# AllanYangZhou/midGPT

Measured on AMD Instinct MI355X. Metric: tokens_per_sec, higher is better.
Workload: dtype bf16; 1 GPU; model=openwebtext_xl-gpt-1311M, global_batch=128, seq_len=1024, parallelism=dp1, g_accum_iters=2, remat=False

## Files before the change

midgpt_amd/models/gpt.py:

```python
from __future__ import annotations

import contextlib
import math
import os

import torch
import torch.nn as nn
import torch.nn.functional as F

from midgpt_amd import ops
from midgpt_amd.config import GPTConfig
from midgpt_amd.ops.reference import rope_tables


_SCOPES = os.environ.get("MIDGPT_SCOPES") == "1"


def _scope(name):
    return torch.profiler.record_function(name) if _SCOPES \
        else contextlib.nullcontext()


def _init_linear_(w: torch.Tensor, in_features: int, generator=None):
    nn.init.trunc_normal_(w, mean=0.0, std=1.0, a=-2.0, b=2.0, generator=generator)
    with torch.no_grad():
        w.mul_(1.0 / math.sqrt(in_features))


class Linear(nn.Module):

    def __init__(self, in_features: int, out_features: int, generator=None):
        super().__init__()
        self.weight = nn.Parameter(torch.empty(out_features, in_features))
        _init_linear_(self.weight, in_features, generator)

    def forward(self, x):
        return F.linear(x, self.weight.to(x.dtype))


class CausalSelfAttention(nn.Module):
    def __init__(self, config: GPTConfig, generator=None):
        super().__init__()
        D, H = config.n_embd, config.n_head
        assert D % H == 0
        self.n_head, self.n_embd = H, D
        self.head_dim = D // H
        self.c_attn = Linear(D, 3 * D, generator)
        self.c_proj = Linear(D, D, generator)
        self.q_ln_weight = nn.Parameter(torch.ones(self.head_dim))
        self.k_ln_weight = nn.Parameter(torch.ones(self.head_dim))
        self.dropout = config.dropout
        self.attn_dropout = nn.Dropout(config.dropout)
        self.resid_dropout = nn.Dropout(config.dropout)

    def forward(self, x, sin, cos):
        with _scope("causal_sa"):
            return self._forward(x, sin, cos)

    def _forward(self, x, sin, cos):
        B, T, D = x.shape
        qkv = self.c_attn(x).view(B, T, 3, self.n_head, self.head_dim)
        if (self.dropout > 0.0 and self.training
                and os.environ.get("MIDGPT_ATTN_DROPOUT_REF") == "1"):
            from midgpt_amd.ops import reference as refops
            q, k, v = ops.qkv_prep(qkv, self.q_ln_weight, self.k_ln_weight,
                                   sin[:T], cos[:T])
            o = refops.causal_attention(q, k, v, self.dropout, True)
            o = o.transpose(1, 2).reshape(B, T, D)
        else:
            o = ops.qkv_attention(qkv, self.q_ln_weight, self.k_ln_weight,
                                  sin[:T], cos[:T],
                                  self.dropout if self.training else 0.0)
        return self.resid_dropout(self.c_proj(o))


class MLP(nn.Module):
    def __init__(self, config: GPTConfig, generator=None):
        super().__init__()
        D = config.n_embd
        self.c_fc = Linear(D, 4 * D, generator)
        self.c_proj = Linear(4 * D, D, generator)
        self.dropout = nn.Dropout(config.dropout)

    def forward(self, x):
        with _scope("mlp"):
            if (x.is_cuda and x.dtype == torch.bfloat16 and ops.have_ext()
                    and os.environ.get("MIDGPT_FUSED_MLP") == "1"):
                return self.dropout(ops.fused_mlp(x, self.c_fc.weight,
                                                  self.c_proj.weight))
            if os.environ.get("MIDGPT_GELU_HIP") == "1":
                return self.dropout(self.c_proj(ops.gelu(self.c_fc(x))))
            return self.dropout(
                self.c_proj(F.gelu(self.c_fc(x), approximate="tanh")))


class Block(nn.Module):

    def __init__(self, config: GPTConfig, generator=None):
        super().__init__()
        self.attn = CausalSelfAttention(config, generator)
        self.mlp = MLP(config, generator)

    def forward(self, x, sin, cos):
        with _scope("block"):
            x = x + self.attn(ops.rmsnorm(x, None, 1e-6), sin, cos)
            x = x + self.mlp(ops.rmsnorm(x, None, 1e-6))
            return x

    def forward_pending(self, x, pending, sin, cos):
        with _scope("block"):
            if pending is None:
                h = ops.rmsnorm(x, None, 1e-6)
            else:
                x, h = ops.add_rmsnorm(x, pending, 1e-6)
            x, h = ops.add_rmsnorm(x, self.attn(h, sin, cos), 1e-6)
            return x, self.mlp(h)


class GPT(nn.Module):
# ... 56 lines not shown
```

midgpt_amd/ops/__init__.py:

```python
from __future__ import annotations

import math
import os

import torch

from midgpt_amd.ops import ref_backend

_C = None
_C_ERR: str | None = None

BACKEND_API = (
    "rmsnorm_fwd", "rmsnorm_bwd", "qkv_prep_fwd", "qkv_prep_bwd",
    "attn_fwd", "attn_bwd", "attn_fwd_dropout", "attn_bwd_dropout",
    "gelu_fwd", "gelu_bwd", "embedding_bwd", "ce_fwd", "ce_bwd",
    "adamw_step", "kv_append", "attn_decode",
)
RAGGED_API = ("kv_append_ragged", "attn_decode_ragged")
SAMPLING_API = ("sample_tokens",)
SLOT_API = ("kv_append_slots", "attn_decode_slots", "sample_tokens_rows")
PAGED_API = ("kv_append_paged", "attn_decode_paged", "kv_store_paged")


def _try_load_ext():
    global _C, _C_ERR
    if _C is not None:
        return _C
    try:
        import importlib
        _C = importlib.import_module("midgpt_amd.ops._C")
    except Exception as e:
        _C_ERR = repr(e)
        _C = None
    return _C


_try_load_ext()


def have_ext() -> bool:
    return _C is not None


def _use_hip(*tensors) -> bool:
    on_gpu = any(t.is_cuda for t in tensors if isinstance(t, torch.Tensor))
    if not on_gpu:
        return False
    if os.environ.get("MIDGPT_FORCE_REF") == "1":
        return False
    if _C is None:
        raise RuntimeError(
            "midgpt_amd HIP extension (midgpt_amd/ops/_C) is not built but a GPU "
            f"tensor reached a hot op. Build it with __graft_entry__.build(). "
            f"Import error: {_C_ERR}")
    return True


def _backend(*tensors):
    return _C if _use_hip(*tensors) else ref_backend


class _RMSNorm(torch.autograd.Function):
    @staticmethod
    def forward(ctx, x, weight, eps):
        shp = x.shape
        x2d = x.reshape(-1, shp[-1])
        y, invrms = _backend(x).rmsnorm_fwd(x2d.contiguous(), weight, eps)
        ctx.save_for_backward(x2d, invrms, *( [weight] if weight is not None else [] ))
        ctx.eps = eps
        ctx.has_w = weight is not None
        return y.reshape(shp)

    @staticmethod
    def backward(ctx, dy):
        saved = ctx.saved_tensors
        x2d, invrms = saved[0], saved[1]
        weight = saved[2] if ctx.has_w else None
        dy2d = dy.reshape(x2d.shape)
        dx, dw = _backend(x2d).rmsnorm_bwd(dy2d.contiguous(), x2d.contiguous(),
                                           weight, invrms, ctx.eps)
        return dx.reshape(dy.shape), dw, None


def rmsnorm(x, weight=None, eps: float = 1e-6):
    return _RMSNorm.apply(x, weight, eps)


def glue_unfused() -> bool:
    return os.environ.get("MIDGPT_GLUE_UNFUSED") == "1"


class _AddRMSNorm(torch.autograd.Function):
    @staticmethod
    def forward(ctx, x, r, eps):
        shp = x.shape
        D = shp[-1]
        s, y, invrms = _C.add_rmsnorm_fwd(x.reshape(-1, D).contiguous(),
                                          r.reshape(-1, D).contiguous(), eps)
        ctx.save_for_backward(s, invrms)
        ctx.set_materialize_grads(False)
        return s.view(shp), y.view(shp)

    @staticmethod
    def backward(ctx, ds, dy):
# ... 454 lines not shown
        if x.dtype != torch.bfloat16 or x.numel() % 8:
            impl = ref_backend
        return impl.gelu_fwd(x.contiguous())

    @staticmethod
    def backward(ctx, dy):
        (x,) = ctx.saved_tensors
        impl = _backend(x)
        if x.dtype != torch.bfloat16 or x.numel() % 8:
            impl = ref_backend
        return impl.gelu_bwd(dy.contiguous(), x.contiguous())


def gelu(x):
    return _Gelu.apply(x)


class _Embedding(torch.autograd.Function):
    @staticmethod
    def forward(ctx, idx, weight):
        ctx.save_for_backward(idx)
        ctx.V = weight.shape[0]
        return weight[idx]

    @staticmethod
    def backward(ctx, dy):
        (idx,) = ctx.saved_tensors
        dy2d = dy.reshape(-1, dy.shape[-1])
        impl = _backend(dy)
        if dy.dtype != torch.bfloat16:
            impl = ref_backend
        return None, impl.embedding_bwd(dy2d.contiguous(), idx.reshape(-1), ctx.V)


def embedding(idx, weight):
    return _Embedding.apply(idx, weight)


class _CrossEntropy(torch.autograd.Function):
    @staticmethod
    def forward(ctx, logits, targets):
        loss_sum, lse = _backend(logits).ce_fwd(logits, targets)
        ctx.save_for_backward(logits, targets, lse)
        return loss_sum / logits.shape[0]

    @staticmethod
    def backward(ctx, dloss):
        logits, targets, lse = ctx.saved_tensors
        dlogits = _backend(logits).ce_bwd(logits, targets, lse,
                                          dloss.float().reshape(1))
        return dlogits, None


def cross_entropy(logits, targets):
    return _CrossEntropy.apply(logits, targets)


class _FusedMLP(torch.autograd.Function):
    @staticmethod
    def forward(ctx, x2d, w1, w2):
        h = torch.mm(x2d, w1.t())
        g = torch.nn.functional.gelu(h, approximate="tanh")
        y = torch.mm(g, w2.t())
        ctx.save_for_backward(x2d, w1, w2, h, g)
        return y

    @staticmethod
    def backward(ctx, dy):
        x2d, w1, w2, h, g = ctx.saved_tensors
        dy = dy.contiguous()
        dh = _C.matmul_dgelu(dy, w2, h)
        dw2 = torch.mm(dy.t(), g)
        dx = torch.mm(dh, w1)
        dw1 = torch.mm(dh.t(), x2d)
        return dx, dw1, dw2


def fused_mlp(x, w1, w2):
    shp = x.shape
    y = _FusedMLP.apply(x.reshape(-1, shp[-1]).contiguous(), w1, w2)
    return y.reshape(*shp[:-1], w2.shape[0])


def adamw_step(master: torch.Tensor, grad: torch.Tensor, m: torch.Tensor,
               v: torch.Tensor, out_bf16: torch.Tensor | None,
               *, lr: float, beta1: float, beta2: float, eps: float,
               wd_over_peak_lr: float, grad_scale: float, clip_norm: float,
               sq_sum: torch.Tensor, step: int):
    _backend(master).adamw_step(master, grad, m, v,
                                out_bf16 if out_bf16 is not None
                                else master.new_empty(0, dtype=torch.bfloat16),
                                out_bf16 is not None, sq_sum,
                                lr, beta1, beta2, eps, wd_over_peak_lr,
                                grad_scale, clip_norm, step)
```

midgpt_amd/ops/csrc/bindings.cpp:

```cpp
#include <torch/extension.h>
#include <hip/hip_runtime.h>
#include <c10/hip/HIPGuard.h>
#include <c10/hip/HIPStream.h>

#include <algorithm>
#include <climits>
#include <type_traits>
#include <vector>

static hipStream_t cur_stream() { return c10::hip::getCurrentHIPStream().stream(); }

template <typename... P, typename... A>
static void launch(void (*kernel)(P...), dim3 grid, int block, size_t smem, A... args) {
  if (grid.x == 0 || grid.y == 0 || grid.z == 0) return;
  if (smem > 64 * 1024) {
    hipError_t e = hipFuncSetAttribute(reinterpret_cast<const void*>(kernel),
                                       hipFuncAttributeMaxDynamicSharedMemorySize, (int)smem);
    TORCH_CHECK(e == hipSuccess, "cannot raise dynamic LDS to ", smem, " bytes: ",
                hipGetErrorString(e));
  }
  hipLaunchKernelGGL(kernel, grid, dim3(block), smem, cur_stream(), static_cast<P>(args)...);
  hipError_t e = hipGetLastError();
  TORCH_CHECK(e == hipSuccess, "HIP launch failed: ", hipGetErrorString(e));
}
// ... 503 lines not shown

std::vector<torch::Tensor> attn_fwd_packed(torch::Tensor q, torch::Tensor k,
                                           torch::Tensor v, double p, int64_t seed) {
  Call c("attn_fwd_packed", q);
  const AttnQK a = attn_qk(c, q, k);
  AttnStrides sv;
  const u16* vp = packed_or_plain_v(c, a, v, &sv);
  auto o = torch::empty({a.B, a.T, a.H, a.C}, q.options());
  auto lse = torch::empty({a.B, a.H, a.T}, q.options().dtype(torch::kFloat));
  attn_fwd_launch(a, vp, sv, fresh<u16>(o), strides_bthc(a.H, a.T, a.C), fresh<float>(lse),
                  drop_if(p, seed));
  return {o, lse};
}

std::vector<torch::Tensor> attn_bwd_packed(torch::Tensor dO, torch::Tensor q,
                                           torch::Tensor k, torch::Tensor v,
                                           torch::Tensor o, torch::Tensor lse,
                                           torch::Tensor dqkv, double p, int64_t seed,
                                           bool stage_do) {
  Call c("attn_bwd_packed", dO);
  const AttnQK a = attn_qk(c, q, k);
  const int B = a.B, H = a.H, T = a.T, C = a.C;
  AttnStrides sv;
  const u16* vp = packed_or_plain_v(c, a, v, &sv);
  u16* dvp = c.bf16_out(dqkv, "dqkv", {B, T, 3, H, C}) + 2L * H * C;
  const u16 *dop = c.bf16(dO, "dO", {B, T, H, C}), *op = c.bf16(o, "o", {B, T, H, C});
  const float* lsep = c.f32(lse, "lse", flat(a.rows()));
  const AttnStrides sdv = strides_qkv_slot(H, T, C), so = strides_bthc(H, T, C);
  torch::Tensor do_copy;
  if (stage_do) do_copy = torch::empty_like(q);
  return attn_bwd_launch(a, dop, so, vp, sv, op, so, lsep, dvp, sdv, drop_if(p, seed),
                         stage_do ? fresh<u16>(do_copy) : nullptr);
}

torch::Tensor embedding_bwd(torch::Tensor dy, torch::Tensor idx, long V) {
  Call c("embedding_bwd", dy);
  const u16* dyp = c.bf16(dy, "dy", {ANY, ANY});
  long N = dy.size(0);
  int D = c.dim(dy, 1);
  const long* ip = c.i64(idx, "idx", {N});
  TORCH_CHECK(D % 8 == 0, "embedding_bwd: D % 8 == 0");
  if (D % 64 == 0) {
    auto sorted_perm = idx.sort();
    auto sorted = std::get<0>(sorted_perm).contiguous();
    auto perm = std::get<1>(sorted_perm).contiguous();
    auto dw = torch::zeros({V, (long)D}, dy.options());
    const int wpb = 4;
    long grid = (N + wpb - 1) / wpb;
    for (int d0 = 0; d0 < D; d0 += 2048)
      launch(embed_bwd_sorted_kernel, grid, wpb * 64, 0, dyp, fresh<long>(sorted),
             fresh<long>(perm), fresh<u16>(dw), N, D, d0);
    return dw;
  }
  auto dw32 = torch::zeros({V, (long)D}, dy.options().dtype(torch::kFloat));
  long grid = std::min(N, (long)4096);
  launch(embed_bwd_scatter_kernel, grid, 256, 0, dyp, ip, fresh<float>(dw32), N, D);
  auto dw = torch::empty({V, (long)D}, dy.options());
  long n = V * (long)D;
  long cgrid = std::min((n / 4 + 255) / 256 + 1, (long)4096);
  launch(f32_to_bf16_kernel, cgrid, 256, 0, fresh<float>(dw32), fresh<u16>(dw), n);
  return dw;
}

torch::Tensor gelu_fwd(torch::Tensor x) {
  Call c("gelu_fwd", x);
  long n = x.numel();
  const u16* xp = c.bf16(x, "x", flat(n));
  TORCH_CHECK(n % 8 == 0, "gelu_fwd: numel % 8 == 0 required");
  auto y = torch::empty_like(x);
  long grid = std::min((n / 8 + 255) / 256 + 1, (long)8192);
  launch(gelu_fwd_bf16, grid, 256, 0, xp, fresh<u16>(y), n);
  return y;
}

torch::Tensor gelu_bwd(torch::Tensor dy, torch::Tensor x) {
  Call c("gelu_bwd", dy);
  long n = x.numel();
  const u16 *xp = c.bf16(x, "x", flat(n)), *dyp = c.bf16(dy, "dy", flat(n));
  TORCH_CHECK(n % 8 == 0, "gelu_bwd: numel % 8 == 0 required");
  auto dx = torch::empty_like(x);
  long grid = std::min((n / 8 + 255) / 256 + 1, (long)8192);
  launch(gelu_bwd_bf16, grid, 256, 0, dyp, xp, fresh<u16>(dx), n);
  return dx;
}

static int64_t decode_caches(const Call& c, const torch::Tensor& k_cache,
                             const torch::Tensor& v_cache, int B, int H, int C, u16** kp,
                             u16** vp, int* pool = nullptr) {
  TORCH_CHECK(C == 64 || C == 128, c.who, ": head dim 64 or 128 (got ", C, ")");
  *kp = c.bf16_out(k_cache, "k_cache", {pool ? ANY : B, H, ANY, C});
  *vp = c.bf16_out(v_cache, "v_cache", k_cache.sizes());
  if (pool) {
    *pool = c.dim(k_cache, 0);
    TORCH_CHECK(*pool >= B, c.who, ": a pool of ", *pool, " slots cannot hold ", B, " rows");
  }
  return k_cache.size(2);
}

static std::vector<int64_t> host_lens(const torch::Tensor& t, int B, const char* who) {
  TORCH_CHECK(!t.is_cuda() && t.dim() == 1 && t.size(0) == B &&
              at::isIntegralType(t.scalar_type(), false),
              who, ": the host copy must be a CPU integer tensor of ", B, " values");
  auto t64 = t.to(torch::kLong).contiguous();
  const int64_t* p = t64.data_ptr<int64_t>();
  return std::vector<int64_t>(p, p + B);
}

struct SlotMap {
  std::vector<int64_t> host;
  const int* dev = nullptr;
  int S = 0;
};
static SlotMap slot_map(const Call& c, const torch::Tensor& slots_dev,
                        const torch::Tensor& slots_host, int B, int64_t S) {
  SlotMap m;
  m.host = host_lens(slots_host, B, c.who);
  TORCH_CHECK(S <= INT_MAX, c.who, ": too many slots");
  std::vector<bool> seen((size_t)std::max<int64_t>(S, 0), false);
  for (int64_t s : m.host) {
    TORCH_CHECK(s >= 0 && s < S, c.who, ": slot ", s, " is outside the pool of ", S);
    TORCH_CHECK(!seen[(size_t)s], c.who, ": slot ", s, " is named twice");
    seen[(size_t)s] = true;
  }
  m.dev = c.i32(slots_dev, "slots_dev", {B});
  m.S = (int)S;
  return m;
}

struct PageTable {
  torch::Tensor host64;
  const int64_t* host = nullptr;
  const int* dev = nullptr;
  int B = 0, P = 0, MP = 0, PS = 0, shift = 0;
  std::vector<int64_t> written;

  int64_t tmax() const { return (int64_t)MP * PS; }
  void cover(const Call& c, int b, int64_t lo, int64_t hi, bool write) {
    for (int64_t j = lo / PS; j * PS < hi; ++j) {
      const int64_t pg = host[(size_t)b * MP + j];
      TORCH_CHECK(pg >= 0 && pg < P, c.who, ": block_table[", b, "][", j, "] = ", pg,
                  " is outside the pool of ", P, " pages");
      if (write) written.push_back(pg);
    }
  }
  void check_writes(const Call& c) {
    std::sort(written.begin(), written.end());
    const auto dup = std::adjacent_find(written.begin(), written.end());
    TORCH_CHECK(dup == written.end(), c.who, ": page ", dup == written.end() ? -1 : *dup,
                " receives writes twice");
  }
};
static PageTable page_table(const Call& c, const torch::Tensor& table_dev,
                            const torch::Tensor& table_host, const torch::Tensor& k_pool,
                            const torch::Tensor& v_pool, int B, int H, int C, u16** kp,
                            u16** vp) {
  PageTable t;
  TORCH_CHECK(C == 64 || C == 128, c.who, ": head dim 64 or 128 (got ", C, ")");
  *kp = c.bf16_out(k_pool, "k_pool", {ANY, H, ANY, C});
  *vp = c.bf16_out(v_pool, "v_pool", k_pool.sizes());
  t.B = B;
  t.P = c.dim(k_pool, 0);
  t.PS = c.dim(k_pool, 2);
  TORCH_CHECK(t.PS >= 16 && t.PS <= 128 && (t.PS & (t.PS - 1)) == 0, c.who,
              ": the page size must be a power of two in [16, 128], got ", t.PS);
  while ((1 << t.shift) < t.PS) ++t.shift;
  TORCH_CHECK(!table_host.is_cuda() && table_host.dim() == 2 && table_host.size(0) == B &&
// ... 320 lines not shown
  auto out = torch::empty({(long)B}, logits.options().dtype(torch::kLong));
  launch(sample_tokens_rows_kernel, B, SAMPLE_THREADS, 0, lp, fresh<long>(out), V, pp);
  return out;
}

torch::Tensor probe_mfma(torch::Tensor A, torch::Tensor B) {
  Call c("probe_mfma", A);
  const float *ap = c.f32(A, "A", {32, 16}), *bp = c.f32(B, "B", {16, 32});
  auto D = torch::zeros({32, 32}, A.options());
  launch(probe_mfma_kernel, 1, 64, 0, ap, bp, fresh<float>(D));
  return D;
}
torch::Tensor probe_pack(torch::Tensor M, torch::Tensor B) {
  Call c("probe_pack", M);
  const float *mp = c.f32(M, "M", {32, 32}), *bp = c.f32(B, "B", {32, 32});
  auto D = torch::zeros({32, 32}, M.options());
  launch(probe_pack_kernel, 1, 64, 0, mp, bp, fresh<float>(D));
  return D;
}

#include "blaslt.inc"

PYBIND11_MODULE(TORCH_EXTENSION_NAME, mod) {
  mod.def("rmsnorm_fwd", &rmsnorm_fwd);
  mod.def("rmsnorm_bwd", &rmsnorm_bwd);
  mod.def("qkv_prep_fwd", &qkv_prep_fwd);
  mod.def("qkv_prep_bwd", &qkv_prep_bwd);
  mod.def("add_rmsnorm_fwd", &add_rmsnorm_fwd);
  mod.def("add_rmsnorm_bwd", &add_rmsnorm_bwd);
  mod.def("qk_prep_fwd", &qk_prep_fwd);
  mod.def("qk_prep_bwd", &qk_prep_bwd);
  mod.def("ce_fwd", &ce_fwd);
  mod.def("ce_bwd", &ce_bwd);
  mod.def("adamw_step", &adamw_step);
  mod.def("attn_fwd", &attn_fwd);
  mod.def("attn_bwd", &attn_bwd);
  mod.def("attn_fwd_dropout", &attn_fwd_dropout);
  mod.def("attn_bwd_dropout", &attn_bwd_dropout);
  mod.def("attn_fwd_packed", &attn_fwd_packed, py::arg("q"), py::arg("k"),
          py::arg("v"), py::arg("p") = 0.0, py::arg("seed") = 0);
  mod.def("attn_bwd_packed", &attn_bwd_packed, py::arg("dO"), py::arg("q"),
          py::arg("k"), py::arg("v"), py::arg("o"), py::arg("lse"),
          py::arg("dqkv"), py::arg("p") = 0.0, py::arg("seed") = 0,
          py::arg("stage_do") = true);
  mod.def("kv_append", &kv_append, py::arg("qkv"), py::arg("qw"), py::arg("kw"),
          py::arg("sin"), py::arg("cos"), py::arg("k_cache"), py::arg("v_cache"),
          py::arg("pos"), py::arg("eps") = 1e-6);
  mod.def("attn_decode", &attn_decode, py::arg("q"), py::arg("k_cache"),
          py::arg("v_cache"), py::arg("kv_len"), py::arg("num_splits") = 0);
  mod.def("kv_append_ragged", &kv_append_ragged, py::arg("qkv"), py::arg("qw"),
          py::arg("kw"), py::arg("sin"), py::arg("cos"), py::arg("k_cache"),
          py::arg("v_cache"), py::arg("pos_dev"), py::arg("pos_host"),
          py::arg("eps") = 1e-6);
  mod.def("attn_decode_ragged", &attn_decode_ragged, py::arg("q"), py::arg("k_cache"),
          py::arg("v_cache"), py::arg("kv_lens_dev"), py::arg("kv_lens_host"),
          py::arg("num_splits") = 0);
  mod.def("kv_append_slots", &kv_append_slots, py::arg("qkv"), py::arg("qw"), py::arg("kw"),
          py::arg("sin"), py::arg("cos"), py::arg("k_cache"), py::arg("v_cache"),
          py::arg("pos_dev"), py::arg("pos_host"), py::arg("slots_dev"),
          py::arg("slots_host"), py::arg("eps") = 1e-6);
  mod.def("attn_decode_slots", &attn_decode_slots, py::arg("q"), py::arg("k_cache"),
          py::arg("v_cache"), py::arg("kv_lens_dev"), py::arg("kv_lens_host"),
          py::arg("slots_dev"), py::arg("slots_host"), py::arg("num_splits") = 0);
  mod.def("kv_append_paged", &kv_append_paged, py::arg("qkv"), py::arg("qw"), py::arg("kw"),
          py::arg("sin"), py::arg("cos"), py::arg("k_pool"), py::arg("v_pool"),
          py::arg("pos_dev"), py::arg("pos_host"), py::arg("block_table_dev"),
          py::arg("block_table_host"), py::arg("eps") = 1e-6);
  mod.def("attn_decode_paged", &attn_decode_paged, py::arg("q"), py::arg("k_pool"),
          py::arg("v_pool"), py::arg("kv_lens_dev"), py::arg("kv_lens_host"),
          py::arg("block_table_dev"), py::arg("block_table_host"), py::arg("num_splits") = 0);
  mod.def("kv_store_paged", &kv_store_paged, py::arg("k"), py::arg("v"), py::arg("k_pool"),
          py::arg("v_pool"), py::arg("lens_dev"), py::arg("lens_host"),
          py::arg("block_table_dev"), py::arg("block_table_host"));
  mod.def("attn_decode_auto_splits", &attn_decode_auto_splits, py::arg("rows"),
          py::arg("kv_len"), py::arg("cus"));
  mod.def("sample_tokens", &sample_tokens, py::arg("logits"), py::arg("inv_t"),
          py::arg("top_k"), py::arg("seed"), py::arg("step"));
  mod.def("sample_tokens_rows", &sample_tokens_rows, py::arg("logits"), py::arg("params_dev"),
          py::arg("inv_t"), py::arg("top_k"), py::arg("seeds"), py::arg("steps"),
          py::arg("rows"));
  mod.def("embedding_bwd", &embedding_bwd);
  mod.def("gelu_fwd", &gelu_fwd);
  mod.def("gelu_bwd", &gelu_bwd);
  mod.def("lt_probe", &lt_probe);
  mod.def("matmul_dgelu", &matmul_dgelu);
  mod.def("probe_mfma", &probe_mfma);
  mod.def("probe_pack", &probe_pack);
}
```

midgpt_amd/ops/csrc/ext.hip:

```cpp
#include "norms.hip"
#include "ce.hip"
#include "adamw.hip"
#include "attention.hip"
#include "decode.hip"
#include "embedding.hip"
#include "gelu.hip"
#include "sampling.hip"
#include "probe.hip"
#include "bindings.cpp"
```

midgpt_amd/ops/ref_backend.py:

```python
from __future__ import annotations

import math

import torch

from midgpt_amd.ops import reference as ref


def rmsnorm_fwd(x2d, weight, eps):
    xf = x2d.float()
    invrms = torch.rsqrt(xf.pow(2).mean(dim=-1) + eps)
    y = xf * invrms[:, None]
    if weight is not None:
        y = y * weight.float()
    return y.to(x2d.dtype), invrms


def rmsnorm_bwd(dy2d, x2d, weight, invrms, eps):
    xf = x2d.float()
    dyf = dy2d.float()
    g = dyf * weight.float() if weight is not None else dyf
    r = invrms[:, None]
    mean_xg = (xf * g).mean(dim=-1, keepdim=True)
    dx = (r * g - xf * r.pow(3) * mean_xg).to(x2d.dtype)
# ... 347 lines not shown
    best = score.max(dim=-1, keepdim=True).values
    idx = torch.arange(V, device=logits.device).expand(B, V)
    tok = torch.where(score == best, idx, V).min(dim=-1).values
    return tok.clamp_(max=V - 1)


def sample_tokens_rows(logits, params_dev, inv_t, top_k, seeds, steps, rows):
    if logits.dim() != 2 or logits.shape[1] < 1:
        raise RuntimeError(f"sample_tokens_rows: logits must be (B, V), got {tuple(logits.shape)}")
    B, V = logits.shape
    who = "sample_tokens_rows"
    if inv_t.is_cuda or inv_t.shape != (B,) or inv_t.dtype != torch.float32:
        raise RuntimeError(f"{who}: inv_t must be a CPU float32 tensor of {B} values")
    inv_t = [float(x) for x in inv_t.tolist()]
    top_k, seeds = _host_lens(top_k, B, who), _host_lens(seeds, B, who)
    steps, rows = _host_lens(steps, B, who), _host_lens(rows, B, who)
    for b in range(B):
        if not (math.isfinite(inv_t[b]) and inv_t[b] >= 0):
            raise RuntimeError(f"{who}: inv_t must be finite and > 0, or 0 for a "
                               f"greedy row, got {inv_t[b]}")
        if top_k[b] < 0:
            raise RuntimeError(f"{who}: top_k >= 0 required (0: all), got {top_k[b]}")
        if not (0 <= steps[b] < 1 << 32 and 0 <= rows[b] < 1 << 32):
            raise RuntimeError(f"{who}: step and row must be in [0, 2^32), got "
                               f"{steps[b]}, {rows[b]}")
    out = []
    for b in range(B):
        if inv_t[b] == 0:
            out.append(_sample_from_words(logits[b:b + 1], 1.0, 0, None))
        else:
            words = ref.sample_words(1, V, seeds[b], steps[b], row0=rows[b])
            out.append(_sample_from_words(logits[b:b + 1], inv_t[b], top_k[b], words))
    return torch.cat(out) if out else torch.empty(0, dtype=torch.int64, device=logits.device)


def gelu_fwd(x):
    return torch.nn.functional.gelu(x, approximate="tanh")


def gelu_bwd(dy, x):
    xf = x.float()
    c0, c1 = 0.7978845608028654, 0.044715
    inner = c0 * (xf + c1 * xf ** 3)
    t = torch.tanh(inner)
    dg = 0.5 * (1 + t) + 0.5 * xf * (1 - t * t) * c0 * (1 + 3 * c1 * xf ** 2)
    return (dy.float() * dg).to(x.dtype)


def embedding_bwd(dy2d, idx, V):
    dw32 = torch.zeros(V, dy2d.shape[-1], dtype=torch.float32, device=dy2d.device)
    dw32.index_add_(0, idx, dy2d.float())
    return dw32.to(dy2d.dtype)


def ce_fwd(logits, targets):
    lf = logits.float()
    lse = torch.logsumexp(lf, dim=-1)
    picked = lf.gather(1, targets[:, None]).squeeze(1)
    return (lse - picked).sum(), lse


def ce_bwd(logits, targets, lse, gscale):
    N = logits.shape[0]
    lf = logits.float()
    p = torch.exp(lf - lse[:, None])
    p.scatter_add_(1, targets[:, None],
                   -torch.ones(N, 1, device=p.device, dtype=p.dtype))
    return (p * (gscale / N)).to(logits.dtype)


def adamw_step(master, grad, m, v, out_bf16, write_bf16, sq_sum, lr, beta1, beta2,
               eps, wd_over_peak_lr, grad_scale, clip_norm, step):
    gnorm = float(sq_sum.float().sqrt()) * grad_scale
    clip_coef = grad_scale * min(1.0, clip_norm / (gnorm + 1e-12))
    g = grad * clip_coef
    m.mul_(beta1).add_(g, alpha=1 - beta1)
    v.mul_(beta2).addcmul_(g, g, value=1 - beta2)
    mhat = m / (1 - beta1 ** step)
    vhat = v / (1 - beta2 ** step)
    update = mhat / (vhat.sqrt() + eps) + wd_over_peak_lr * master
    master.add_(update, alpha=-lr)
    if write_bf16:
        out_bf16.copy_(master.to(torch.bfloat16))
```

midgpt_amd/parallel/engine.py:

```python
from __future__ import annotations

import os

import torch

from midgpt_amd import ops
from midgpt_amd.parallel import dist as pdist


class ShardedAdamW:
    def __init__(self, model: torch.nn.Module, *,
                 compute_dtype: torch.dtype = torch.bfloat16,
                 zero: bool = True,
                 beta1: float = 0.9, beta2: float = 0.95,
                 eps: float = 1e-8, weight_decay: float = 1e-4,
                 peak_lr: float = 1e-3, grad_clip: float = 1.0,
                 device: torch.device | None = None,
                 n_buckets: int | None = None):
        self.model = model
        self.beta1, self.beta2, self.eps = beta1, beta2, eps
        self.wd_over_peak = weight_decay / peak_lr
        self.grad_clip = grad_clip
        self.step_count = 0

# ... 7 lines not shown
        self.device = device
        self.compute_dtype = compute_dtype

        self.meta = []
        off = 0
        names = {p: n for n, p in model.named_parameters()}
        for p in params:
            n = p.numel()
            self.meta.append((names[p], tuple(p.shape), off, n))
            off += n
        total = off
        self.total = total
        self.shard_size = (total + self.world - 1) // self.world if self.zero else total
        self.padded = self.shard_size * self.world if self.zero else total
        self.shard_off = self.rank * self.shard_size if self.zero else 0

        if n_buckets is None:
            n_buckets = int(os.environ.get("MIDGPT_ZERO_BUCKETS", "4"))
        S = self.shard_size
        nb = max(1, min(n_buckets, S)) if self.zero else \
            max(1, min(n_buckets, max(1, self.padded // (1 << 20))))
        if self.zero:
            cuts = [S * i // nb for i in range(nb + 1)]
            self.buckets = [(cuts[i] * self.world,
                             (cuts[i + 1] - cuts[i]) * self.world)
                            for i in range(nb)]
            self.pieces = []
            po = 0
            for (o_b, n_b) in self.buckets:
                p_b = n_b // self.world
                self.pieces.append((o_b + self.rank * p_b, p_b, po))
                po += p_b
        else:
            cuts = [self.padded * i // nb for i in range(nb + 1)]
            self.buckets = [(cuts[i], cuts[i + 1] - cuts[i]) for i in range(nb)]
            self.pieces = [(o, n, o) for (o, n) in self.buckets]
        self.n_buckets = len(self.buckets)

        full32 = torch.zeros(self.padded, dtype=torch.float32, device=device)
        for p, (_, _, o, n) in zip(params, self.meta):
            full32[o:o + n].copy_(p.detach().reshape(-1).to(device, torch.float32))
        self.master = self._take_shard(full32)
        self.flat_w = full32.to(compute_dtype)
        del full32
        self._overlap = device.type == "cuda"
        nbuf = 2 if self._overlap else 1
        self.flat_gs = [torch.zeros(self.padded, dtype=compute_dtype,
                                    device=device) for _ in range(nbuf)]
        self._cur = 0
        self.params = params
        for p, (_, shape, o, n) in zip(params, self.meta):
            p.data = self.flat_w[o:o + n].view(shape)
        self._rebind_grads()

        self.m = torch.zeros_like(self.master)
        self.v = torch.zeros_like(self.master)
        self.g32 = torch.zeros_like(self.master)
        self._g16_shards = [torch.empty(self.shard_size, dtype=compute_dtype,
                                        device=device) for _ in range(nbuf)] \
            if self.zero else None
        self._w16_shard = torch.empty(self.shard_size, dtype=compute_dtype,
                                      device=device) if self.zero else None
        if self._overlap:
            self._comm_stream = torch.cuda.Stream(device=device)
            self._pending = []
        if self.world > 1:
            pdist.all_reduce_(torch.zeros(1, device=device))
        self._bucket_params = [0] * self.n_buckets
        self._param_buckets: list[list[int]] = []
        for (_, _, o, n) in self.meta:
            bl = [b for b, (o_b, n_b) in enumerate(self.buckets)
                  if o < o_b + n_b and o + n > o_b]
            self._param_buckets.append(bl)
            for b in bl:
                self._bucket_params[b] += 1
        self._hooks_on = self._overlap and self.n_buckets > 1
        self._counts = list(self._bucket_params)
        self._ready = [False] * self.n_buckets
        self._next_launch = self.n_buckets - 1
        self._launched = [False] * self.n_buckets
        if self._hooks_on:
            for i, p in enumerate(self.params):
                p.register_post_accumulate_grad_hook(self._make_hook(i))

    def _take_shard(self, full: torch.Tensor) -> torch.Tensor:
        if not self.zero:
            return full.clone()
        out = torch.empty(self.shard_size, dtype=full.dtype, device=full.device)
        for (fo, p_b, po) in self.pieces:
            out[po:po + p_b].copy_(full[fo:fo + p_b])
        return out

    def _scatter_shard(self, shard: torch.Tensor, full: torch.Tensor):
        for (fo, p_b, po) in self.pieces:
            full[fo:fo + p_b].copy_(shard[po:po + p_b])

    @property
    def flat_g(self):
        return self.flat_gs[self._cur]

    def _rebind_grads(self):
        cur = self.flat_gs[self._cur]
        for p, (_, shape, o, n) in zip(self.params, self.meta):
            p.grad = cur[o:o + n].view(shape)

    def _make_hook(self, param_idx: int):
        def hook(_p):
            for b in self._param_buckets[param_idx]:
                self._counts[b] -= 1
                if self._counts[b] == 0:
                    self._ready[b] = True
            while self._next_launch >= 0 and self._ready[self._next_launch]:
                self._launch_bucket(self._next_launch)
                self._next_launch -= 1
        return hook

    def _launch_bucket(self, b: int):
        cur = self._cur
        o_b, n_b = self.buckets[b]
        if n_b == 0:
            self._launched[b] = True
            return
        ready = torch.cuda.Event()
        ready.record()
        with torch.cuda.stream(self._comm_stream):
            self._comm_stream.wait_event(ready)
            if self.zero:
                fo, p_b, po = self.pieces[b]
                pdist.reduce_scatter_flat(
                    self.flat_gs[cur][o_b:o_b + n_b],
                    self._g16_shards[cur][po:po + p_b])
            elif self.world > 1:
                pdist.all_reduce_(self.flat_gs[cur][o_b:o_b + n_b])
        self._launched[b] = True

    def _drain(self, buf: int | None = None):
        keep = []
        for done, b in self._pending:
            if buf is not None and b != buf:
                keep.append((done, b))
                continue
            torch.cuda.current_stream().wait_event(done)
            if self.zero:
                self.g32.add_(self._g16_shards[b])
            else:
                self.g32.add_(self.flat_gs[b])
            self.flat_gs[b].zero_()
        self._pending = keep

    def microstep_end(self):
        if not self._overlap:
            for b, (o_b, n_b) in enumerate(self.buckets):
                if n_b == 0:
                    continue
                if self.zero:
                    fo, p_b, po = self.pieces[b]
                    pdist.reduce_scatter_flat(
                        self.flat_gs[0][o_b:o_b + n_b],
                        self._g16_shards[0][po:po + p_b])
                elif self.world > 1:
                    pdist.all_reduce_(self.flat_gs[0][o_b:o_b + n_b])
            if self.zero:
                self.g32.add_(self._g16_shards[0])
            else:
                self.g32.add_(self.flat_gs[0])
            self.flat_gs[0].zero_()
            return
        cur = self._cur
        if self._hooks_on:
            while self._next_launch >= 0:
                self._launch_bucket(self._next_launch)
                self._next_launch -= 1
            self._counts = list(self._bucket_params)
            self._ready = [False] * self.n_buckets
            self._launched = [False] * self.n_buckets
            self._next_launch = self.n_buckets - 1
        else:
            for b in range(self.n_buckets - 1, -1, -1):
                self._launch_bucket(b)
            self._launched = [False] * self.n_buckets
        done = torch.cuda.Event()
        with torch.cuda.stream(self._comm_stream):
            done.record(self._comm_stream)
        self._pending.append((done, cur))
        self._cur = cur ^ 1
        self._drain(buf=self._cur)
        self._rebind_grads()

    def defer_until(self, evt) -> None:
        self._defer_evt = evt

    def step(self, lr: float, g_accum_iters: int = 1) -> torch.Tensor:
        if getattr(self, "_defer_evt", None) is not None:
            torch.cuda.current_stream().wait_event(self._defer_evt)
            self._defer_evt = None
        if self._overlap:
            self._drain()
        scale = 1.0 / (g_accum_iters * self.world)
        sq = self.g32.pow(2).sum()
        if self.zero:
            pdist.all_reduce_(sq)
        self.step_count += 1
        out_view = (self._w16_shard if self.zero else self.flat_w)
        ops.adamw_step(self.master, self.g32, self.m, self.v,
                       out_view if self.compute_dtype == torch.bfloat16 else None,
                       lr=lr, beta1=self.beta1, beta2=self.beta2, eps=self.eps,
                       wd_over_peak_lr=self.wd_over_peak,
                       grad_scale=scale, clip_norm=self.grad_clip,
                       sq_sum=sq, step=self.step_count)
        if self.compute_dtype != torch.bfloat16:
            out_view.copy_(self.master.to(self.compute_dtype))
        if self.zero:
            self._allgather_weights()
        self.g32.zero_()
        return sq

    def _allgather_weights(self):
        for b, (o_b, n_b) in enumerate(self.buckets):
            if n_b == 0:
                continue
            fo, p_b, po = self.pieces[b]
            pdist.all_gather_flat(self.flat_w[o_b:o_b + n_b],
                                  self._w16_shard[po:po + p_b])

    def state_shard(self) -> dict:
        return {
            "master": self.master,
            "m": self.m,
            "v": self.v,
            "step_count": self.step_count,
            "shard_off": self.shard_off,
            "shard_size": self.shard_size,
            "pieces": [[fo, p_b, po] for (fo, p_b, po) in self.pieces],
            "total": self.total,
            "padded": self.padded,
            "world": self.world if self.zero else 1,
        }

    def load_state_full(self, full_master, full_m, full_v, step_count: int):
        def take(t):
            out = torch.zeros(self.padded, dtype=torch.float32)
            k = min(t.numel(), self.padded)
            out[:k] = t.reshape(-1)[:k].float()
            return self._take_shard(out.to(self.device))
        self.master.copy_(take(full_master))
        self.m.copy_(take(full_m))
        self.v.copy_(take(full_v))
        self.step_count = step_count
        self.refresh_weights()

    def refresh_weights(self):
        if self.zero:
            self._w16_shard.copy_(self.master.to(self.compute_dtype))
            self._allgather_weights()
        else:
            self.flat_w.copy_(self.master.to(self.compute_dtype))

    def named_param_manifest(self) -> list[dict]:
        return [{"name": n, "shape": list(s), "offset": o, "numel": k}
                for (n, s, o, k) in self.meta]
```

Baseline: 107,000 tokens/s.

## Keep transposed bf16 weight images for dgrad GEMMs, refreshed by batched transpose kernel

Adds a pre-transposed copy of every Linear weight, kept in one flat buffer and refreshed after each optimizer step by a new batched tiled transpose HIP kernel. A custom autograd function computes the input gradient as dy @ wt.t(), aiming to give the dgrad GEMM a more favorable operand layout than the default transposed-weight path. The cost is an extra copy of the weights in memory (about 2.6 GB for 1.3B params) plus one transpose pass per step.

Measured after the change: 110,100 tokens/s (median of 6 runs). +2.9%, better.

```diff
diff --git a/midgpt_amd/models/gpt.py b/midgpt_amd/models/gpt.py
--- a/midgpt_amd/models/gpt.py
+++ b/midgpt_amd/models/gpt.py
@@ -33,8 +33,13 @@
         super().__init__()
         self.weight = nn.Parameter(torch.empty(out_features, in_features))
         _init_linear_(self.weight, in_features, generator)
+        self.weight_t = None
 
     def forward(self, x):
+        wt = self.weight_t
+        if (wt is not None and torch.is_grad_enabled() and x.is_cuda
+                and x.dtype == torch.bfloat16 and self.weight.dtype == torch.bfloat16):
+            return ops.linear_wt(x, self.weight, wt)
         return F.linear(x, self.weight.to(x.dtype))
 
 
diff --git a/midgpt_amd/ops/__init__.py b/midgpt_amd/ops/__init__.py
--- a/midgpt_amd/ops/__init__.py
+++ b/midgpt_amd/ops/__init__.py
@@ -20,6 +20,7 @@
 SAMPLING_API = ("sample_tokens",)
 SLOT_API = ("kv_append_slots", "attn_decode_slots", "sample_tokens_rows")
 PAGED_API = ("kv_append_paged", "attn_decode_paged", "kv_store_paged")
+TRANSPOSE_API = ("transpose_batched",)
 
 
 def _try_load_ext():
@@ -640,6 +641,48 @@
     return y.reshape(*shp[:-1], w2.shape[0])
 
 
+class _LinearWt(torch.autograd.Function):
+    @staticmethod
+    def forward(ctx, x, w, wt):
+        ctx.save_for_backward(x, wt)
+        return torch.nn.functional.linear(x, w)
+
+    @staticmethod
+    def backward(ctx, dy):
+        x, wt = ctx.saved_tensors
+        dy2d = dy.reshape(-1, dy.shape[-1])
+        dx = dw = None
+        if ctx.needs_input_grad[0]:
+            dx = dy2d.mm(wt.t()).view(x.shape)
+        if ctx.needs_input_grad[1]:
+            dw = dy2d.t().mm(x.reshape(-1, x.shape[-1]))
+        return dx, dw, None
+
+
+def linear_wt(x, w, wt):
+    if wt.shape != (w.shape[1], w.shape[0]) or not (x.dtype == w.dtype == wt.dtype):
+        raise RuntimeError(f"linear_wt: w {tuple(w.shape)} {w.dtype} needs an image "
+                           f"{(w.shape[1], w.shape[0])} of its dtype and x's "
+                           f"({x.dtype}), got {tuple(wt.shape)} {wt.dtype}")
+    return _LinearWt.apply(x, w, wt)
+
+
+TRANSPOSE_TILE = ref_backend.TRANSPOSE_TILE
+
+
+def transpose_table(entries, device=None):
+    rows5, tiles = [], 0
+    for (so, do, r, c) in entries:
+        rows5.append([int(so), int(do), int(r), int(c), tiles])
+        tiles += -(-int(r) // TRANSPOSE_TILE) * -(-int(c) // TRANSPOSE_TILE)
+    host = torch.tensor(rows5, dtype=torch.int64).reshape(-1, 5)
+    return (host if device is None else host.to(device)), host
+
+
+def transpose_batched(src, dst, table_dev, table_host, max_blocks: int = 0):
+    _backend(src).transpose_batched(src, dst, table_dev, table_host, int(max_blocks))
+
+
 def adamw_step(master: torch.Tensor, grad: torch.Tensor, m: torch.Tensor,
                v: torch.Tensor, out_bf16: torch.Tensor | None,
                *, lr: float, beta1: float, beta2: float, eps: float,
diff --git a/midgpt_amd/ops/csrc/bindings.cpp b/midgpt_amd/ops/csrc/bindings.cpp
--- a/midgpt_amd/ops/csrc/bindings.cpp
+++ b/midgpt_amd/ops/csrc/bindings.cpp
@@ -609,6 +609,39 @@
   long grid = std::min((n / 8 + 255) / 256 + 1, (long)8192);
   launch(gelu_bwd_bf16, grid, 256, 0, dyp, xp, fresh<u16>(dx), n);
   return dx;
+}
+
+void transpose_batched(torch::Tensor src, torch::Tensor dst, torch::Tensor table_dev,
+                       torch::Tensor table_host, int64_t max_blocks) {
+  Call c("transpose_batched", src);
+  const int64_t ns = src.numel(), nd = dst.numel();
+  const u16* sp = c.bf16(src, "src", flat(ns));
+  u16* dp = c.bf16_out(dst, "dst", flat(nd));
+  TORCH_CHECK(sp + ns <= dp || dp + nd <= sp, c.who, ": src and dst overlap");
+  TORCH_CHECK(!table_host.is_cuda() && table_host.dim() == 2 && table_host.size(1) == TR_COLS &&
+              table_host.scalar_type() == torch::kLong && table_host.is_contiguous(),
+              c.who, ": the host table must be a contiguous CPU int64 tensor (n, 5)");
+  const int64_t n = table_host.size(0);
+  TORCH_CHECK(n <= INT_MAX, c.who, ": too many matrices");
+  const long* tp = c.i64(table_dev, "table_dev", {n, TR_COLS});
+  const int64_t* h = table_host.data_ptr<int64_t>();
+  int64_t tiles = 0;
+  for (int64_t m = 0; m < n; ++m, h += TR_COLS) {
+    const int64_t so = h[0], d_o = h[1], rows = h[2], cols = h[3];
+    TORCH_CHECK(rows >= 1 && cols >= 1 && rows <= ns && cols <= ns / rows,
+                c.who, ": matrix ", m, " is ", rows, " x ", cols, ", src holds ", ns);
+    const int64_t numel = rows * cols;
+    TORCH_CHECK(so >= 0 && so <= ns - numel, c.who, ": matrix ", m, " at ", so, " leaves src");
+    TORCH_CHECK(d_o >= 0 && numel <= nd && d_o <= nd - numel,
+                c.who, ": image ", m, " at ", d_o, " leaves dst");
+    TORCH_CHECK(h[4] == tiles, c.who, ": tile prefix of matrix ", m, " is ", h[4],
+                ", expected ", tiles);
+    tiles += ((rows + TR_TILE - 1) / TR_TILE) * ((cols + TR_TILE - 1) / TR_TILE);
+  }
+  TORCH_CHECK(max_blocks >= 0, c.who, ": max_blocks must be >= 0");
+  const int64_t cap = max_blocks > 0 ? max_blocks : 2048;
+  launch(transpose_batched_kernel, (unsigned)std::min(tiles, cap), 256, 0, sp, dp, tp, (int)n,
+         (long)tiles);
 }
 
 static int64_t decode_caches(const Call& c, const torch::Tensor& k_cache,
@@ -1095,6 +1128,8 @@
   mod.def("embedding_bwd", &embedding_bwd);
   mod.def("gelu_fwd", &gelu_fwd);
   mod.def("gelu_bwd", &gelu_bwd);
+  mod.def("transpose_batched", &transpose_batched, py::arg("src"), py::arg("dst"),
+          py::arg("table_dev"), py::arg("table_host"), py::arg("max_blocks") = 0);
   mod.def("lt_probe", &lt_probe);
   mod.def("matmul_dgelu", &matmul_dgelu);
   mod.def("probe_mfma", &probe_mfma);
diff --git a/midgpt_amd/ops/csrc/ext.hip b/midgpt_amd/ops/csrc/ext.hip
--- a/midgpt_amd/ops/csrc/ext.hip
+++ b/midgpt_amd/ops/csrc/ext.hip
@@ -6,5 +6,6 @@
 #include "embedding.hip"
 #include "gelu.hip"
 #include "sampling.hip"
+#include "transpose.hip"
 #include "probe.hip"
 #include "bindings.cpp"
diff --git a/midgpt_amd/ops/csrc/transpose.hip b/midgpt_amd/ops/csrc/transpose.hip
--- /dev/null
+++ b/midgpt_amd/ops/csrc/transpose.hip
@@ -0,0 +1,67 @@
+#include "common.h"
+
+#define TR_TILE 64
+#define TR_STRIDE_W 33
+#define TR_STRIDE (2 * TR_STRIDE_W)
+#define TR_COLS 5
+
+__global__ __launch_bounds__(256) void transpose_batched_kernel(
+    const u16* __restrict__ src, u16* __restrict__ dst, const long* __restrict__ tab,
+    int n_mat, long n_tiles) {
+  __shared__ unsigned tile_w[TR_TILE * TR_STRIDE_W];
+  u16* tile = reinterpret_cast<u16*>(tile_w);
+  const int tid = threadIdx.x;
+
+  for (long t = blockIdx.x; t < n_tiles; t += gridDim.x) {
+    int lo = 0, hi = n_mat - 1;
+    while (lo < hi) {
+      const int mid = (lo + hi + 1) >> 1;
+      if (tab[mid * TR_COLS + 4] <= t) lo = mid;
+      else hi = mid - 1;
+    }
+    const long* e = tab + lo * TR_COLS;
+    const long rows = e[2], cols = e[3];
+    const long local = t - e[4];
+    const long tiles_c = (cols + TR_TILE - 1) / TR_TILE;
+    const long r0 = (local / tiles_c) * TR_TILE, c0 = (local % tiles_c) * TR_TILE;
+    const u16* s = src + e[0] + r0 * cols + c0;
+    u16* d = dst + e[1] + c0 * rows + r0;
+    const bool vec = r0 + TR_TILE <= rows && c0 + TR_TILE <= cols && rows % 8 == 0 &&
+                     cols % 8 == 0 && reinterpret_cast<uintptr_t>(s) % 16 == 0 &&
+                     reinterpret_cast<uintptr_t>(d) % 16 == 0;
+    if (vec) {
+#pragma unroll
+      for (int p = 0; p < 2; ++p) {
+        const int idx = tid + p * 256;
+        const int r = idx >> 3, v = idx & 7;
+        const u16x8 x = *reinterpret_cast<const u16x8*>(s + r * cols + v * 8);
+        unsigned* w = tile_w + r * TR_STRIDE_W + v * 4;
+#pragma unroll
+        for (int k = 0; k < 4; ++k) w[k] = (unsigned)x[2 * k] | ((unsigned)x[2 * k + 1] << 16);
+      }
+      __syncthreads();
+      const int lane = tid & 63, wave = tid >> 6;
+      const int j = (lane >> 5) * 4 + (lane & 3);
+#pragma unroll
+      for (int p = 0; p < 2; ++p) {
+        const int c = p * 32 + wave * 8 + ((lane >> 2) & 7);
+        u16x8 o;
+#pragma unroll
+        for (int i = 0; i < 8; ++i) o[i] = tile[(8 * j + i) * TR_STRIDE + c];
+        *reinterpret_cast<u16x8*>(d + c * rows + 8 * j) = o;
+      }
+    } else {
+      const int nr = (int)min((long)TR_TILE, rows - r0), nc = (int)min((long)TR_TILE, cols - c0);
+      for (int idx = tid; idx < TR_TILE * TR_TILE; idx += 256) {
+        const int r = idx >> 6, c = idx & 63;
+        if (r < nr && c < nc) tile[r * TR_STRIDE + c] = s[r * cols + c];
+      }
+      __syncthreads();
+      for (int idx = tid; idx < TR_TILE * TR_TILE; idx += 256) {
+        const int c = idx >> 6, r = idx & 63;
+        if (r < nr && c < nc) d[c * rows + r] = tile[r * TR_STRIDE + c];
+      }
+    }
+    __syncthreads();
+  }
+}
diff --git a/midgpt_amd/ops/ref_backend.py b/midgpt_amd/ops/ref_backend.py
--- a/midgpt_amd/ops/ref_backend.py
+++ b/midgpt_amd/ops/ref_backend.py
@@ -453,3 +453,29 @@
     master.add_(update, alpha=-lr)
     if write_bf16:
         out_bf16.copy_(master.to(torch.bfloat16))
+
+
+TRANSPOSE_TILE = 64
+
+
+def transpose_batched(src, dst, table_dev, table_host, max_blocks=0):
+    who = "transpose_batched"
+    if src.dim() != 1 or dst.dim() != 1 or src.dtype != dst.dtype:
+        raise RuntimeError(f"{who}: src and dst must be flat buffers of one dtype")
+    t = table_host
+    if t.is_cuda or t.dim() != 2 or t.shape[1] != 5 or t.dtype != torch.int64:
+        raise RuntimeError(f"{who}: the host table must be a CPU int64 tensor (n, 5)")
+    if tuple(table_dev.shape) != tuple(t.shape):
+        raise RuntimeError(f"{who}: the device table must be {tuple(t.shape)}")
+    tiles = 0
+    for m, (so, do, rows, cols, prefix) in enumerate(t.tolist()):
+        if rows < 1 or cols < 1 or so < 0 or so + rows * cols > src.numel():
+            raise RuntimeError(f"{who}: matrix {m} ({rows} x {cols} at {so}) leaves src")
+        if do < 0 or do + rows * cols > dst.numel():
+            raise RuntimeError(f"{who}: image {m} at {do} leaves dst")
+        if prefix != tiles:
+            raise RuntimeError(f"{who}: tile prefix of matrix {m} is {prefix}, "
+                               f"expected {tiles}")
+        tiles += -(-rows // TRANSPOSE_TILE) * -(-cols // TRANSPOSE_TILE)
+        dst[do:do + rows * cols].view(cols, rows).copy_(
+            src[so:so + rows * cols].view(rows, cols).t())
diff --git a/midgpt_amd/parallel/engine.py b/midgpt_amd/parallel/engine.py
--- a/midgpt_amd/parallel/engine.py
+++ b/midgpt_amd/parallel/engine.py
@@ -113,6 +113,35 @@
         if self._hooks_on:
             for i, p in enumerate(self.params):
                 p.register_post_accumulate_grad_hook(self._make_hook(i))
+        self._init_dgrad_images()
+
+    def _init_dgrad_images(self):
+        from midgpt_amd.models.gpt import Linear
+        self.flat_wt = None
+        if (self.device.type != "cuda" or self.compute_dtype != torch.bfloat16
+                or not ops.have_ext()
+                or os.environ.get("MIDGPT_DGRAD_WT", "1") == "0"):
+            return
+        offset = {id(p): (o, shape) for p, (_, shape, o, _) in zip(self.params, self.meta)}
+        linears = [m for m in self.model.modules()
+                   if isinstance(m, Linear) and id(m.weight) in offset]
+        if not linears:
+            return
+        entries, off = [], 0
+        for m in linears:
+            o, (rows, cols) = offset[id(m.weight)]
+            entries.append((o, off, rows, cols))
+            off += -(-rows * cols // 8) * 8
+        self.flat_wt = torch.empty(off, dtype=self.compute_dtype, device=self.device)
+        self._wt_table_dev, self._wt_table = ops.transpose_table(entries, self.device)
+        for m, (_, do, rows, cols) in zip(linears, entries):
+            m.weight_t = self.flat_wt[do:do + rows * cols].view(cols, rows)
+        self.refresh_dgrad_images()
+
+    def refresh_dgrad_images(self):
+        if self.flat_wt is not None:
+            ops.transpose_batched(self.flat_w, self.flat_wt, self._wt_table_dev,
+                                  self._wt_table)
 
     def _take_shard(self, full: torch.Tensor) -> torch.Tensor:
         if not self.zero:
@@ -243,6 +272,7 @@
             out_view.copy_(self.master.to(self.compute_dtype))
         if self.zero:
             self._allgather_weights()
+        self.refresh_dgrad_images()
         self.g32.zero_()
         return sq
 
@@ -286,6 +316,7 @@
             self._allgather_weights()
         else:
             self.flat_w.copy_(self.master.to(self.compute_dtype))
+        self.refresh_dgrad_images()
 
     def named_param_manifest(self) -> list[dict]:
         return [{"name": n, "shape": list(s), "offset": o, "numel": k}
```
